# dmMaze/comic-text-detector

Measured on NVIDIA H100. Metric: pages/sec @1024x1024 synthetic, higher is better.
Workload: dtype fp16

## Files before the change

### comic-text-detector_b200/binding.py

```python
import collections
import ctypes as C
import os

import numpy as np

_HERE = os.path.dirname(os.path.abspath(__file__))
LIB_PATH = os.path.join(_HERE, "libctd_b200.so")
MAX_SRC = 3
ABI_VERSION = 3
PREC_FP16_TC, PREC_FP32_SIMT, PREC_FP16_SIMT, PREC_SPLIT_TC = 0, 1, 2, 3


class CtdOp(C.Structure):
    _fields_ = [("kind", C.c_int32), ("n_src", C.c_int32), ("src_buf", C.c_int32 * MAX_SRC),
                ("src_coff", C.c_int32 * MAX_SRC), ("src_c", C.c_int32 * MAX_SRC), ("dst_buf", C.c_int32),
                ("dst_coff", C.c_int32), ("cout", C.c_int32), ("cout_pad", C.c_int32), ("ksize", C.c_int32),
                ("stride", C.c_int32), ("act", C.c_int32), ("residual", C.c_int32), ("aux", C.c_int32),
                ("w16_off", C.c_int64), ("w32_off", C.c_int64), ("b_off", C.c_int64), ("p_off", C.c_int64)]


class CtdBufDesc(C.Structure):
    _fields_ = [("channels", C.c_int32), ("down", C.c_int32)]


class CtdConfig(C.Structure):
# ... 51 lines not shown
                ("event", C.c_void_p)]


class CtdNetOutput(C.Structure):
    _fields_ = [("blks", C.c_void_p), ("blks_stride_r", C.c_int64), ("blks_stride_c", C.c_int64),
                ("mask", C.c_void_p), ("mask_stride_h", C.c_int64), ("mask_stride_w", C.c_int64),
                ("lines", C.c_void_p), ("lines_stride_h", C.c_int64), ("lines_stride_w", C.c_int64),
                ("rows", C.c_int32), ("blks_on_device", C.c_int32), ("mask_on_device", C.c_int32),
                ("lines_on_device", C.c_int32), ("event", C.c_void_p)]


EXPORTS = ["ctd_create", "ctd_destroy", "ctd_last_error", "ctd_forward", "ctd_get_net_outputs", "ctd_get_mask_u8",
           "ctd_get_detections", "ctd_get_db_components", "ctd_last_forward_ms", "ctd_last_launch_count",
           "ctd_debug_read_buffer", "ctd_debug_write_buffer", "ctd_connected_components", "ctd_nms",
           "ctd_timer_start", "ctd_timer_stop", "ctd_profile_forward", "ctd_get_text_lines", "ctd_seg_represent",
           "ctd_refine_mask", "ctd_collect", "ctd_join", "ctd_resize_linear_u8", "ctd_debug_run_ops",
           "ctd_get_nms_status", "ctd_group_output", "ctd_detect_page", "ctd_results_layout", "ctd_submit_full",
           "ctd_device_arena", "ctd_region_plan", "ctd_transform_regions", "ctd_pages_plan", "ctd_submit_pages",
           "ctd_collect_regions", "ctd_collect_device", "ctd_forward_tensor", "ctd_jpeg_probe",
           "ctd_jpeg_decoder_create", "ctd_jpeg_decoder_destroy", "ctd_jpeg_decode", "ctd_debug_postprocess",
           "ctd_png_encoder_create", "ctd_png_encoder_destroy", "ctd_png_encode", "ctd_png_probe",
           "ctd_png_decoder_create", "ctd_png_decoder_destroy", "ctd_png_decode", "ctd_png_decoder_stats",
           "ctd_refine_plan", "ctd_submit_refine", "ctd_submit_regions", "ctd_debug_read_slot", "ctd_submit_outputs",
           "ctd_preprocess_pages", "ctd_submit_outputs_dtype", "ctd_forward_tensor_f16", "ctd_nms_dtype"]
PRE_F32_NCHW, PRE_F16_NCHW, PRE_U8_NHWC = 0, 1, 2
DTYPE_F32, DTYPE_F16 = 0, 1

_lib = None


class CtdError(RuntimeError):
# ... 39 lines not shown
    lib.ctd_debug_read_buffer.argtypes = [vp, i32, vp, C.c_size_t]
    lib.ctd_debug_write_buffer.argtypes = [vp, i32, vp, i32, i32, i32]
    lib.ctd_connected_components.argtypes = [vp, vp, i32, i32, vp, vp, i32, vp]
    lib.ctd_nms.argtypes = [vp, vp, i32, C.c_float, C.c_float, vp, vp]
    lib.ctd_nms_dtype.argtypes = [vp, vp, i32, i32, C.c_float, C.c_float, vp, vp]
    lib.ctd_get_text_lines.argtypes = [vp, vp, vp, vp]
    lib.ctd_seg_represent.argtypes = [vp, vp, i32, i32, C.c_float, vp, vp, vp]
    lib.ctd_refine_mask.argtypes = [vp, vp, vp, i32, i32, vp, i32, i32, vp]
    lib.ctd_timer_start.argtypes = [vp]
    lib.ctd_timer_stop.argtypes = [vp, C.POINTER(C.c_float)]
    lib.ctd_profile_forward.argtypes = [vp, vp, i32, i32, i32, i32, vp, i32]
    lib.ctd_collect.argtypes = [vp, i32]
    lib.ctd_join.argtypes = [vp, vp]
    lib.ctd_resize_linear_u8.argtypes = [vp, vp, i32, i32, i32, vp, i32, i32]
    lib.ctd_debug_run_ops.argtypes = [vp, vp, i32, i32, i32, i32, i32]
    lib.ctd_debug_postprocess.argtypes = [vp, vp, vp, i32, i32, i32]
    lib.ctd_get_nms_status.argtypes = [vp, vp, C.POINTER(i32)]
    lib.ctd_group_output.argtypes = [vp, vp, i32, vp, i32, i32, i32, vp, i32, vp, i32, vp, i32, vp, i32, C.POINTER(i32)]
    lib.ctd_detect_page.argtypes = [vp, vp, i32, i32, i32, i32, i32, i32, vp, vp, vp, i32, vp, i32, vp, i32, C.POINTER(i32)]
    lib.ctd_results_layout.argtypes = [vp, C.POINTER(CtdResultsLayout)]
    lib.ctd_submit_full.argtypes = [vp, i32, vp, i32, i32, i32, i32, i32, vp]
    lib.ctd_device_arena.argtypes = [vp, i32, C.POINTER(vp), C.POINTER(vp)]
    lib.ctd_region_plan.argtypes = [vp, i32, i32, i32, i32, vp, C.POINTER(C.c_size_t)]
    lib.ctd_transform_regions.argtypes = [vp, vp, i32, i32, i32, vp, i32, vp, C.c_size_t]
    lib.ctd_pages_plan.argtypes = [vp, i32, i32, i32, C.POINTER(C.c_size_t), C.POINTER(C.c_size_t)]
    lib.ctd_submit_pages.argtypes = [vp, i32, vp, i32, i32, i32, vp, vp, i32, i32, i32, i32, vp]
    lib.ctd_collect_regions.argtypes = [vp, i32, C.POINTER(vp), C.POINTER(i32), C.POINTER(vp), C.POINTER(vp),
                                        C.POINTER(C.c_size_t)]
    lib.ctd_collect_device.argtypes = [vp, i32, vp]
    lib.ctd_refine_plan.argtypes = [vp, i32, vp, vp, vp, vp, C.POINTER(C.c_size_t), C.POINTER(C.c_size_t)]
# ... 605 lines not shown
    def join(self, other):
        self._ck(self.lib.ctd_join(self.h, other.h))

    def debug_write(self, tensor, arr, n, h, w):
        arr = np.ascontiguousarray(arr, np.float32)
        ch = self.program.bufs[tensor["buf"]][0]
        assert arr.shape == (n, h // tensor["down"], w // tensor["down"], ch), arr.shape
        self._ck(self.lib.ctd_debug_write_buffer(self.h, tensor["buf"], _ptr(arr), n, h, w))

    def debug_run_ops(self, first, last, n, h, w, pages=None):
        if pages is not None:
            pages = np.ascontiguousarray(pages, dtype=np.uint8)
        self._ck(self.lib.ctd_debug_run_ops(self.h, _ptr(pages), n, h, w, first, last))
        self.shape = (n, h, w)

    def debug_read_slot(self, slot, plane, offset, nbytes):
        out = np.empty((nbytes,), np.uint8)
        self._ck(self.lib.ctd_debug_read_slot(self.h, slot, plane, offset, _ptr(out), nbytes))
        return out

    def debug_postprocess(self, blks, lines):
        blks = np.ascontiguousarray(blks, np.float32)
        lines = np.ascontiguousarray(lines, np.float32)
        n, c, h, w = lines.shape
        assert c == 2 and blks.shape == (n, 3 * ((h // 8) * (w // 8) + (h // 16) * (w // 16) + (h // 32) * (w // 32)),
                                         5 + self.nc), (blks.shape, lines.shape)
        self._ck(self.lib.ctd_debug_postprocess(self.h, _ptr(blks), _ptr(lines), n, h, w))
        self.shape = (n, h, w)

    def transform_regions(self, page, plan, out=None, page_shape=None):
# ... 34 lines not shown
```

### comic-text-detector_b200/csrc/conv_tc.cu

```cuda
#include <cstdlib>
#include <cstring>
#include <cuda.h>
#include <cuda_fp16.h>
#include <cuda_runtime.h>

#include "kernels.h"
#include "ptx.cuh"

namespace ctd {

constexpr int kTileW = 16;
constexpr int kThreads = 384;

template <int BN, int TH>
struct TcCfg {
  static constexpr int kABytes = TH * kTileW * 128;
  static constexpr int kBBytes = BN * 128;
  static constexpr int kStages = TH == 8 ? (BN >= 128 ? 5 : (BN >= 64 ? 8 : 10))
                                         : (BN >= 128 ? 3 : (BN >= 64 ? 4 : (BN >= 32 ? 5 : 6)));
  static constexpr int kBoxN = BN < 64 ? BN : 64;
  static constexpr int kBoxBytes = 8 * TH * kBoxN * 2;
  static constexpr int kStgBytes = (BN / kBoxN) * kBoxBytes;
  static constexpr int kBiasFloats = 512;
  static constexpr size_t kSmem = 1024 + size_t(kStages) * (kABytes + kBBytes) + 2 * kStgBytes + 256 + kBiasFloats * 4;
  static_assert(kSmem <= 227 * 1024, "conv_tc_kernel: shared memory");
  static_assert(kBoxBytes % 1024 == 0, "conv_tc_kernel: store boxes must keep the 1024-byte swizzle alignment");
};

template <int ACT>
__device__ __forceinline__ float apply_act(float v) {
  if constexpr (ACT == CTD_ACT_SILU) return __fdividef(v, 1.0f + exp_neg_fast(v));
  else if constexpr (ACT == CTD_ACT_LEAKY) return fmaxf(v, 0.1f * v);
  else if constexpr (ACT == CTD_ACT_RELU) return fmaxf(v, 0.f);
  else if constexpr (ACT == CTD_ACT_SIGMOID) return __fdividef(1.0f, 1.0f + exp_neg_fast(v));
  else return v;
}

template <int ACT>
__device__ __forceinline__ float apply_act_precise(float v) {
  if constexpr (ACT == CTD_ACT_SILU) return v / (1.0f + expf(-v));
  else if constexpr (ACT == CTD_ACT_LEAKY) return fmaxf(v, 0.1f * v);
  else if constexpr (ACT == CTD_ACT_RELU) return fmaxf(v, 0.f);
  else if constexpr (ACT == CTD_ACT_SIGMOID) return 1.0f / (1.0f + expf(-v));
  else return v;
}

template <int BN>
__device__ __forceinline__ void wgmma_bn(float (&d)[BN / 2], uint64_t ad, uint64_t bd, uint32_t acc) {
  if constexpr (BN == 128) wgmma_n128(d, ad, bd, acc);
  else if constexpr (BN == 64) wgmma_n64(d, ad, bd, acc);
  else if constexpr (BN == 32) wgmma_n32(d, ad, bd, acc);
  else wgmma_n16(d, ad, bd, acc);
}

template <int BN, int TH, int ACT, bool RES>
__device__ __forceinline__ void stage_f16(const float (&acc)[BN / 2], const float* __restrict__ bias_s, uint32_t stg,
                                          int m, int warp4, int lane) {
  using Cfg = TcCfg<BN, TH>;
  constexpr uint32_t kRowBytes = Cfg::kBoxN * 2;
  const int q = lane >> 3;
  const uint32_t pixrow = uint32_t(m * 64 + warp4 * 16 + (q & 1) * 8 + (lane & 7));
#pragma unroll
  for (int j = 0; j < BN / 8; j += 2) {
    const int col = (j + (q >> 1)) * 8;
    const uint32_t off = pixrow * kRowBytes + uint32_t(col % Cfg::kBoxN) * 2;
    const uint32_t addr = stg + uint32_t(col / Cfg::kBoxN) * Cfg::kBoxBytes +
                          (off ^ (((off >> 7) & (kRowBytes / 16 - 1)) << 4));
    uint32_t r[4];
    if constexpr (RES) ldmatrix_x4(addr, r);
#pragma unroll
    for (int i = 0; i < 4; ++i) {
      const int c = (j + (i >> 1)) * 8 + (lane & 3) * 2;
      float f0 = apply_act<ACT>(acc[j * 4 + 2 * i] + bias_s[c]);
      float f1 = apply_act<ACT>(acc[j * 4 + 2 * i + 1] + bias_s[c + 1]);
      if constexpr (RES) {
        __half2 h;
        memcpy(&h, &r[i], 4);
        const float2 rv = __half22float2(h);
        f0 = __fadd_rn(f0, rv.x);
        f1 = __fadd_rn(f1, rv.y);
      }
      const __half2 o = __floats2half2_rn(f0, f1);
      memcpy(&r[i], &o, 4);
    }
    stmatrix_x4(addr, r);
  }
}

template <int ACT>
__device__ __forceinline__ void epi_pair_f32(float v0, float v1, const float* __restrict__ bias_s, int col,
                                             float* __restrict__ out, int ncols, bool residual) {
  if (col >= ncols) return;
  float f0 = apply_act_precise<ACT>(v0 + bias_s[col]);
  float f1 = apply_act_precise<ACT>(v1 + bias_s[col + 1]);
  if (col + 1 < ncols) {
    if (residual) {
      const float2 r = *reinterpret_cast<const float2*>(out + col);
      f0 += r.x;
      f1 += r.y;
    }
    *reinterpret_cast<float2*>(out + col) = make_float2(f0, f1);
// ... 493 lines not shown
```

### comic-text-detector_b200/csrc/engine.cu

```cuda
#include <cuda.h>
#include <cuda_fp16.h>
#include <cuda_runtime.h>
#include <stdarg.h>
#include <stdio.h>
#include <string.h>

#include <algorithm>
#include <cstdlib>
#include <map>
#include <string>
#include <tuple>
#include <vector>

#include "engine.h"

using namespace ctd;

namespace {
thread_local std::string g_create_error;
}

int ctd_fail(ctd_handle* h, int code, const char* fmt, ...) {
  char buf[512];
  va_list ap;
// ... 131 lines not shown
  CKC(cudaEventCreate(&h->ev1));
  CKC(cudaEventCreate(&h->tev0));
  CKC(cudaEventCreate(&h->tev1));
  {
    void* fn = nullptr;
    cudaDriverEntryPointQueryResult qres;
    CKC(cudaGetDriverEntryPoint("cuTensorMapEncodeTiled", &fn, cudaEnableDefault, &qres));
    if (!fn || qres != cudaDriverEntryPointSuccess) {
      ctd_fail(h, CTD_E_CUDA, "cuTensorMapEncodeTiled not available from the driver");
      return bail(CTD_E_CUDA);
    }
    h->enc = reinterpret_cast<PFN_encodeTiled>(fn);
  }
  CKC(conv_tc_init());
  CKC(conv_ends_init());
  h->blob_bytes = blob_bytes;
  CKC(cudaMalloc(&h->d_blob, blob_bytes));
  CKC(cudaMemcpy(h->d_blob, blob, blob_bytes, cudaMemcpyHostToDevice));
  const size_t nb = size_t(cfg->max_batch), mh = cfg->max_h, mw = cfg->max_w;
  h->d_buf.assign(n_bufs, nullptr);
  for (int i = 0; i < n_bufs; ++i) {
    const size_t bytes = nb * (mh / bufs[i].down) * (mw / bufs[i].down + 4) * bufs[i].channels * h->elem;
    CKC(cudaMalloc(&h->d_buf[i], bytes));
    CKC(cudaMemset(h->d_buf[i], 0, bytes));
  }
  if (cfg->precision == CTD_PREC_SPLIT_TC) {
    h->d_buf16.assign(n_bufs, nullptr);
    for (int i = 0; i < n_bufs; ++i) {
      const size_t bytes = 2 * nb * (mh / bufs[i].down) * (mw / bufs[i].down + 4) * bufs[i].channels * 2;
      CKC(cudaMalloc(&h->d_buf16[i], bytes));
// ... 110 lines not shown
  p.det_stride = h->detect_prm[i][0];
  for (int k = 0; k < 6; ++k) p.anchor_wh[k] = h->detect_prm[i][1 + k];
}

static bool runs_on_tensor_cores(int precision, int kind) {
  switch (precision) {
    case CTD_PREC_SPLIT_TC: return is_gemm(kind);
    case CTD_PREC_FP16_TC: return is_gemm(kind) || kind == CTD_OP_STEM || kind == CTD_OP_SEG_TAIL;
    default: return false;
  }
}

static int build_plans(ctd_handle* h, int n, int ph, int pw, ShapePlan& sp) {
  sp.tc.resize(h->ops.size());
  sp.ends.resize(h->ops.size());
  const bool split = h->cfg.precision == CTD_PREC_SPLIT_TC;
  for (size_t i = 0; i < h->ops.size(); ++i) {
    const ctd_op& op = h->ops[i];
    if (!runs_on_tensor_cores(h->cfg.precision, op.kind)) continue;
    const float* bias = reinterpret_cast<const float*>(h->d_blob + op.b_off);
    const char* e = nullptr;
    if (op.kind == CTD_OP_STEM) {
      const bool f16 = sp.input == INPUT_F32;
      e = conv_ends_plan_stem(sp.ends[i], h->enc, f16 ? static_cast<const void*>(h->in_stage.p) : h->d_pages, f16, n,
                              ph, pw, h->d_blob + op.w16_off, bias, static_cast<__half*>(h->d_buf[op.dst_buf]),
                              h->bufs[op.dst_buf].channels, op.dst_coff, op.cout, op.act);
    } else if (op.kind == CTD_OP_SEG_TAIL) {
      if (op.cout_pad != 16) return ctd_fail(h, CTD_E_INVALID, "op %zu: seg tail needs cout_pad 16", i);
      const ctd_bufdesc& sb = h->bufs[op.src_buf[0]];
      e = conv_ends_plan_seg(sp.ends[i], h->enc, static_cast<const __half*>(h->d_buf[op.src_buf[0]]), sb.channels,
                             op.src_coff[0], op.src_c[0], n, ph / sb.down, pw / sb.down, h->d_blob + op.w16_off,
                             h->d_mask, h->d_mask_u8);
    } else {
      ConvGeom g;
      if (int rc = op_geom(h, op, n, ph, pw, g)) return rc;
      const void* src[CTD_MAX_SRC];
      int coff[CTD_MAX_SRC];
      for (int s = 0; s < op.n_src; ++s) {
        src[s] = (split ? h->d_buf16 : h->d_buf)[op.src_buf[s]];
        coff[s] = op.src_coff[s];
      }
      const void* w = split ? h->d_wsplit + h->wsplit_off[i] : h->d_blob + op.w16_off;
      __half* dst = op.kind == CTD_OP_DETECT ? nullptr : static_cast<__half*>(h->d_buf[op.dst_buf]);
      e = conv_tc_plan(sp.tc[i], h->enc, g, src, coff, w, bias, dst, split);
      if (op.kind == CTD_OP_DETECT) set_detect(h, i, ph, pw, sp.tc[i].p);
    }
    if (e) return ctd_fail(h, CTD_E_INVALID, "op %zu: %s", i, e);
  }
  return CTD_OK;
}

template <typename T>
static int run_op_simt(ctd_handle* h, size_t i, int n, int ph, int pw) {
  const ctd_op& op = h->ops[i];
  ConvSimtParams p;
  memset(&p, 0, sizeof(p));
  if (int rc = op_geom(h, op, n, ph, pw, p.g)) return rc;
  for (int k = 0; k < op.n_src; ++k)
    p.src[k] = static_cast<char*>(h->d_buf[op.src_buf[k]]) + size_t(op.src_coff[k]) * sizeof(T);
// ... 55 lines not shown
  else if (op.kind == CTD_OP_AVGPOOL2 || op.kind == CTD_OP_UPSAMPLE2) c = op.src_c[0];
  if (buf < 0 || c <= 0) return CTD_OK;
  const ctd_bufdesc& b = h->bufs[buf];
  const size_t npix = size_t(n) * (ph / b.down) * (pw / b.down);
  __half* hi = static_cast<__half*>(h->d_buf16[buf]) + coff;
  CK(split_planes_launch(static_cast<const float*>(h->d_buf[buf]) + coff, hi, hi + npix * b.channels, npix, c, b.channels,
                         h->stream));
  ++*cnt;
  return CTD_OK;
}

static int run_one_op(ctd_handle* h, size_t i, int n, int ph, int pw, const ShapePlan& sp, int* cnt) {
  const ctd_op& op = h->ops[i];
  const ConvTcPlan& tc = sp.tc[i];
  int rc = CTD_OK;
  if (tc.block_n || sp.ends[i].kind != ctd::CTD_END_NONE) {
    const cudaError_t e = tc.block_n ? conv_tc_launch(tc, h->stream) : conv_ends_launch(sp.ends[i], h->stream);
    if (e != cudaSuccess) rc = ctd_fail(h, CTD_E_CUDA, "tensor-core op %zu: %s", i, cudaGetErrorString(e));
  } else if (is_gemm(op.kind)) {
    rc = h->elem == 4 ? run_op_simt<float>(h, i, n, ph, pw) : run_op_simt<__half>(h, i, n, ph, pw);
  } else {
    rc = h->elem == 4 ? run_op_thin<float>(h, op, n, ph, pw, sp.input) : run_op_thin<__half>(h, op, n, ph, pw, sp.input);
  }
  ++*cnt;
  if (rc || h->d_buf16.empty()) return rc;
  return split_written_slice(h, op, n, ph, pw, cnt);
}

int launch_nms(ctd_handle* h, int n, int ph, int pw, cudaStream_t s, int* cnt, const int32_t* half) {
  CK(nms_launch(h->d_blks, n, rows_per_image(ph, pw), h->cfg.nc, h->cfg.conf_thresh, h->cfg.nms_thresh, h->nms, h->d_det,
                h->d_det_count, s, half));
  *cnt += kNmsLaunches;
// ... 432 lines not shown
  if (!h) return CTD_E_INVALID;
  if (first_op < 0 || last_op >= int(h->ops.size()) || first_op > last_op) return ctd_fail(h, CTD_E_INVALID, "bad op range");
  ShapePlan* sp = nullptr;
  if (int rc = find_plan(h, n, ph, pw, &sp)) return rc;
  if (pages) CK(cudaMemcpyAsync(h->d_pages, pages, size_t(n) * ph * pw * 3, cudaMemcpyHostToDevice, h->stream));
  int cnt = 0;
  for (int i = first_op; i <= last_op; ++i)
    if (int rc = run_one_op(h, size_t(i), n, ph, pw, *sp, &cnt)) return rc;
  CK(cudaStreamSynchronize(h->stream));
  h->n = n; h->ph = ph; h->pw = pw;
  h->have_forward = true;
  h->last_launches = cnt;
  return CTD_OK;
}

extern "C" int ctd_debug_postprocess(ctd_handle* h, const float* blks, const float* lines, int32_t n, int32_t ph,
                                     int32_t pw) {
  if (!h || !blks || !lines) return CTD_E_INVALID;
  if (h->cfg.debug_skip_postproc) return ctd_fail(h, CTD_E_INVALID, "ctd_debug_postprocess needs the full pipeline");
  ShapePlan* sp = nullptr;
  if (int rc = find_plan(h, n, ph, pw, &sp)) return rc;
  const size_t hw = size_t(ph) * pw;
  CK(cudaMemcpyAsync(h->d_blks, blks, size_t(n) * rows_per_image(ph, pw) * (5 + h->cfg.nc) * 4, cudaMemcpyHostToDevice,
                     h->stream));
  CK(cudaMemcpyAsync(h->d_lines, lines, size_t(n) * hw * 2 * 4, cudaMemcpyHostToDevice, h->stream));
  for (int i = 0; i < n; ++i)
    CK(binarize_launch(h->d_lines + size_t(i) * 2 * hw, hw, h->cfg.db_thresh, h->d_bitmap + size_t(i) * hw, h->stream));
  int cnt = 0;
  if (int rc = launch_nms(h, n, ph, pw, h->stream, &cnt)) return rc;
  if (int rc = launch_db_post(h, n, ph, pw, h->stream, &cnt)) return rc;
// ... 79 lines not shown
```

### comic-text-detector_b200/csrc/engine.h

```cpp
#pragma once
#include <cuda.h>
#include <cuda_runtime.h>
#include <stdint.h>

#include <math.h>

#include <algorithm>
#include <array>
#include <condition_variable>
#include <deque>
#include <map>
#include <mutex>
#include <optional>
#include <string>
#include <thread>
#include <tuple>
#include <vector>

#include "kernels.h"

using ctd::ConvTcPlan;
using ctd::ConvEndsPlan;
using ctd::NmsWorkspace;
using ctd::PFN_encodeTiled;

struct ArenaLayout {
  size_t det, cnt, nl, lb, ls, lc, a_bytes, refined, blocks, blocks_stride, rec_off, lines_off, dist_off, total;
};

struct BlockSection {
  size_t rec_off, lines_off, dist_off, stride;
};
inline BlockSection block_section_layout() {
  auto al = [](size_t v) { return (v + 255) / 256 * 256; };
  BlockSection b;
  b.rec_off = 64;
  b.lines_off = b.rec_off + al(size_t(CTD_MAX_BLOCKS) * sizeof(ctd_block));
// ... 113 lines not shown
struct RegionJob {
  std::vector<ctd::RegionDev> regs;
  std::vector<ctd::RegionTile> tiles;
  size_t out_bytes = 0;
  int add(const ctd_region* plan, int n, const ctd::RegionPage& pg, long long out_base);
  size_t table_bytes() const;
  void write_tables(char* dst) const;
};

enum { INPUT_U8 = 0, INPUT_F32 = 1 };

struct ShapePlan {
  int input = INPUT_U8;
  std::vector<ConvTcPlan> tc;
  std::vector<ConvEndsPlan> ends;
  cudaGraphExec_t graph = nullptr;
  int launches = 0;
};
struct ctd_handle {
  ctd_config cfg{};
  std::vector<ctd_op> ops;
  std::vector<ctd_bufdesc> bufs;
  std::vector<std::array<float, 7>> detect_prm;
  std::string err;
  cudaStream_t stream = nullptr;
  cudaEvent_t ev0 = nullptr, ev1 = nullptr, tev0 = nullptr, tev1 = nullptr;
  std::vector<cudaEvent_t> op_events;
  PFN_encodeTiled enc = nullptr;
  char* d_blob = nullptr;
  size_t blob_bytes = 0;
// ... 16 lines not shown
  void* d_segrep_scratch = nullptr;
  DevBuf refine_scratch;
  DevBuf cc_scratch;
  DevBuf io_scratch;
  int16_t* d_line_boxes = nullptr;
  float* d_line_scores = nullptr;
  int32_t* d_line_count = nullptr;
  void* d_nms_ws = nullptr;
  NmsWorkspace nms{};
  std::map<std::tuple<int, int, int, int>, ShapePlan> plans;
  DevBuf in_stage;
  cudaEvent_t ev_tin = nullptr, ev_tout = nullptr;
  cudaStream_t copy_in = nullptr, copy_out = nullptr;
  Slot slot[2];
  bool overlap = false;
  cudaStream_t side = nullptr, side2 = nullptr;
  cudaEvent_t ev_fork = nullptr, ev_join = nullptr, ev_fork2 = nullptr, ev_join2 = nullptr;
  cudaEvent_t ev_xjoin = nullptr;
  std::vector<char> db_ancestor;
  ArenaLayout layout{};
  cudaStream_t post = nullptr;
  size_t pipe_pinned_cap = 0;
  std::thread pipe_thread;
  std::mutex pipe_mu;
  std::condition_variable pipe_cv, pipe_done_cv;
  std::deque<PipeJob> pipe_queue;
  bool pipe_quit = false;
  int host_threads = 4;
  size_t pg_gather_off = 0;
  size_t pg_out_off = 0, pg_half_off = 0, pg_flag_off = 0;
// ... 24 lines not shown
```

### comic-text-detector_b200/csrc/kernels.h

```cpp
#pragma once
#include <cuda.h>
#include <cuda_fp16.h>
#include <cuda_runtime.h>
#include <stdint.h>

#include "../../include/ctd_b200.h"

namespace ctd {

constexpr int kMaxTaps = 9;

constexpr float kSplitLoScale = 2048.0f;
constexpr float kSplitLoUnscale = 1.0f / 2048.0f;
constexpr int kMaxPhases = 4;

struct ConvGeom {
  int n_img;
  int gh, gw;
  int dst_h, dst_w;
  int out_mul;
  int n_phase;
  int taps;
  int cin_total;
  int k_total;
// ... 40 lines not shown
  int block_n;
  int tile_h;
  dim3 grid;
  size_t smem_bytes;
};

typedef CUresult (*PFN_encodeTiled)(CUtensorMap*, CUtensorMapDataType, cuuint32_t, void*, const cuuint64_t*,
                                    const cuuint64_t*, const cuuint32_t*, const cuuint32_t*, CUtensorMapInterleave,
                                    CUtensorMapSwizzle, CUtensorMapL2promotion, CUtensorMapFloatOOBfill);

const char* conv_tc_plan(ConvTcPlan& plan, PFN_encodeTiled enc, const ConvGeom& g, const void* const src_ptr[],
                         const int src_coff[], const void* w16, const float* bias, __half* dst, int split = 0);
cudaError_t conv_tc_launch(const ConvTcPlan& plan, cudaStream_t s);
cudaError_t conv_tc_init();

enum { CTD_END_NONE = 0, CTD_END_STEM = 1, CTD_END_SEG = 2, CTD_END_STEM_F16 = 3 };
struct alignas(64) ConvEndsParams {
  CUtensorMap a_map;
  CUtensorMap b_map;
  CUtensorMap d_map;
  int n_img, gh, gw;
  int tiles_x, tiles_y;
  const float* bias;
  float* mask_f32;
  uint8_t* mask_u8;
};
struct ConvEndsPlan {
  ConvEndsParams p;
  int kind = CTD_END_NONE;
  dim3 grid;
// ... 148 lines not shown
```

### include/ctd_b200.h

```cpp
#ifndef CTD_B200_H_
#define CTD_B200_H_

#include <stddef.h>
#include <stdint.h>

#ifdef __cplusplus
extern "C" {
#endif

#define CTD_ABI_VERSION 3
#if defined(__GNUC__)
#define CTD_API __attribute__((visibility("default")))
#else
#define CTD_API
#endif

#define CTD_OK 0
#define CTD_E_INVALID (-1)
#define CTD_E_CUDA (-2)
#define CTD_E_NO_DEVICE (-3)
#define CTD_E_SHAPE (-4)
#define CTD_E_CAPACITY (-5)


// ... 86 lines not shown

CTD_API int ctd_get_text_lines(ctd_handle* h, int16_t* boxes, float* scores, int32_t* counts);

CTD_API int ctd_resize_linear_u8(ctd_handle* h, const uint8_t* src, int32_t sh, int32_t sw, int32_t channels, uint8_t* dst,
                                 int32_t dh, int32_t dw);

CTD_API int ctd_join(ctd_handle* h, ctd_handle* other);

CTD_API int ctd_last_forward_ms(ctd_handle* h, float* ms);
CTD_API int ctd_last_launch_count(ctd_handle* h, int32_t* launches);
CTD_API int ctd_debug_read_buffer(ctd_handle* h, int32_t buf, float* out, size_t out_elems);
CTD_API int ctd_debug_write_buffer(ctd_handle* h, int32_t buf, const float* in, int32_t n, int32_t ph, int32_t pw);

CTD_API int ctd_debug_run_ops(ctd_handle* h, const uint8_t* pages, int32_t n, int32_t ph, int32_t pw, int32_t first_op,
                              int32_t last_op);

CTD_API int ctd_debug_postprocess(ctd_handle* h, const float* blks, const float* lines, int32_t n, int32_t ph, int32_t pw);

CTD_API int ctd_debug_read_slot(ctd_handle* h, int32_t slot, int32_t plane, size_t offset, uint8_t* out, size_t bytes);

CTD_API int ctd_timer_start(ctd_handle* h);
CTD_API int ctd_timer_stop(ctd_handle* h, float* ms);
CTD_API int ctd_profile_forward(ctd_handle* h, const uint8_t* pages, int32_t n, int32_t ph, int32_t pw,
                                int32_t pages_on_device, float* op_ms, int32_t cap);

CTD_API int ctd_connected_components(ctd_handle* h, const uint8_t* img, int32_t ih, int32_t iw, int32_t* labels,
                             int32_t* stats, int32_t stats_cap, int32_t* n_labels);

CTD_API int ctd_seg_represent(ctd_handle* h, const float* pred, int32_t ih, int32_t iw, float thresh, int16_t* boxes,
                              float* scores, int32_t* count);
// ... 220 lines not shown
```

Baseline: 1149.

## Add persistent warp-specialized pointwise conv kernel with weights resident in shared memory

Adds a dedicated 1x1 convolution kernel that loads the full weight slice for its output-channel block into shared memory once, then runs persistent CTAs. Two producer warps stream activation tiles through TMA rings feeding two consumer warpgroups that use wgmma, with a TMA-store epilogue. Eligible 1x1 convs go to it by default (can be disabled with an env var) and the shared epilogue helpers move into a common header. The goal is to avoid reloading weights per tile and to overlap loads with MMA. The cost is a larger shared-memory footprint and one CTA per SM, and layers that don't meet the size or alignment checks fall back to the old kernel.

Result: no change. 1158 (median of 6 runs) (+0.8%).

```diff
diff --git a/comic-text-detector_b200/binding.py b/comic-text-detector_b200/binding.py
--- a/comic-text-detector_b200/binding.py
+++ b/comic-text-detector_b200/binding.py
@@ -9,6 +9,7 @@
 MAX_SRC = 3
 ABI_VERSION = 3
 PREC_FP16_TC, PREC_FP32_SIMT, PREC_FP16_SIMT, PREC_SPLIT_TC = 0, 1, 2, 3
+KERNEL_CUDA_CORES, KERNEL_CONV_TC, KERNEL_ENDS, KERNEL_CONV_PW = 0, 1, 2, 3
 
 
 class CtdOp(C.Structure):
@@ -90,7 +91,7 @@
            "ctd_get_detections", "ctd_get_db_components", "ctd_last_forward_ms", "ctd_last_launch_count",
            "ctd_debug_read_buffer", "ctd_debug_write_buffer", "ctd_connected_components", "ctd_nms",
            "ctd_timer_start", "ctd_timer_stop", "ctd_profile_forward", "ctd_get_text_lines", "ctd_seg_represent",
-           "ctd_refine_mask", "ctd_collect", "ctd_join", "ctd_resize_linear_u8", "ctd_debug_run_ops",
+           "ctd_refine_mask", "ctd_collect", "ctd_join", "ctd_resize_linear_u8", "ctd_debug_run_ops", "ctd_debug_op_kernel",
            "ctd_get_nms_status", "ctd_group_output", "ctd_detect_page", "ctd_results_layout", "ctd_submit_full",
            "ctd_device_arena", "ctd_region_plan", "ctd_transform_regions", "ctd_pages_plan", "ctd_submit_pages",
            "ctd_collect_regions", "ctd_collect_device", "ctd_forward_tensor", "ctd_jpeg_probe",
@@ -160,6 +161,7 @@
     lib.ctd_join.argtypes = [vp, vp]
     lib.ctd_resize_linear_u8.argtypes = [vp, vp, i32, i32, i32, vp, i32, i32]
     lib.ctd_debug_run_ops.argtypes = [vp, vp, i32, i32, i32, i32, i32]
+    lib.ctd_debug_op_kernel.argtypes = [vp, i32, i32, i32, i32, C.POINTER(i32), C.POINTER(i32)]
     lib.ctd_debug_postprocess.argtypes = [vp, vp, vp, i32, i32, i32]
     lib.ctd_get_nms_status.argtypes = [vp, vp, C.POINTER(i32)]
     lib.ctd_group_output.argtypes = [vp, vp, i32, vp, i32, i32, i32, vp, i32, vp, i32, vp, i32, vp, i32, C.POINTER(i32)]
@@ -795,6 +797,11 @@
         self._ck(self.lib.ctd_debug_run_ops(self.h, _ptr(pages), n, h, w, first, last))
         self.shape = (n, h, w)
 
+    def debug_op_kernel(self, op, n, h, w):
+        kernel, bn = C.c_int32(), C.c_int32()
+        self._ck(self.lib.ctd_debug_op_kernel(self.h, n, h, w, op, C.byref(kernel), C.byref(bn)))
+        return kernel.value, bn.value
+
     def debug_read_slot(self, slot, plane, offset, nbytes):
         out = np.empty((nbytes,), np.uint8)
         self._ck(self.lib.ctd_debug_read_slot(self.h, slot, plane, offset, _ptr(out), nbytes))
diff --git a/comic-text-detector_b200/csrc/conv_epi.cuh b/comic-text-detector_b200/csrc/conv_epi.cuh
--- /dev/null
+++ b/comic-text-detector_b200/csrc/conv_epi.cuh
@@ -0,0 +1,68 @@
+#pragma once
+#include <cstring>
+#include <cuda_fp16.h>
+
+#include "kernels.h"
+#include "ptx.cuh"
+
+namespace ctd {
+
+template <int ACT>
+__device__ __forceinline__ float apply_act(float v) {
+  if constexpr (ACT == CTD_ACT_SILU) return __fdividef(v, 1.0f + exp_neg_fast(v));
+  else if constexpr (ACT == CTD_ACT_LEAKY) return fmaxf(v, 0.1f * v);
+  else if constexpr (ACT == CTD_ACT_RELU) return fmaxf(v, 0.f);
+  else if constexpr (ACT == CTD_ACT_SIGMOID) return __fdividef(1.0f, 1.0f + exp_neg_fast(v));
+  else return v;
+}
+
+template <int BN>
+__device__ __forceinline__ void wgmma_bn(float (&d)[BN / 2], uint64_t ad, uint64_t bd, uint32_t acc) {
+  if constexpr (BN == 128) wgmma_n128(d, ad, bd, acc);
+  else if constexpr (BN == 64) wgmma_n64(d, ad, bd, acc);
+  else if constexpr (BN == 32) wgmma_n32(d, ad, bd, acc);
+  else wgmma_n16(d, ad, bd, acc);
+}
+
+template <int BN, int TH>
+struct StgCfg {
+  static constexpr int kBoxN = BN < 64 ? BN : 64;
+  static constexpr int kBoxBytes = 8 * TH * kBoxN * 2;
+  static constexpr int kBytes = (BN / kBoxN) * kBoxBytes;
+};
+
+template <int BN, int TH, int ACT, bool RES>
+__device__ __forceinline__ void stage_f16(const float (&acc)[BN / 2], const float* __restrict__ bias_s, uint32_t stg,
+                                          int m, int warp4, int lane) {
+  using Cfg = StgCfg<BN, TH>;
+  constexpr uint32_t kRowBytes = Cfg::kBoxN * 2;
+  const int q = lane >> 3;
+  const uint32_t pixrow = uint32_t(m * 64 + warp4 * 16 + (q & 1) * 8 + (lane & 7));
+#pragma unroll
+  for (int j = 0; j < BN / 8; j += 2) {
+    const int col = (j + (q >> 1)) * 8;
+    const uint32_t off = pixrow * kRowBytes + uint32_t(col % Cfg::kBoxN) * 2;
+    const uint32_t addr = stg + uint32_t(col / Cfg::kBoxN) * Cfg::kBoxBytes +
+                          (off ^ (((off >> 7) & (kRowBytes / 16 - 1)) << 4));
+    uint32_t r[4];
+    if constexpr (RES) ldmatrix_x4(addr, r);
+#pragma unroll
+    for (int i = 0; i < 4; ++i) {
+      const int c = (j + (i >> 1)) * 8 + (lane & 3) * 2;
+      float f0 = apply_act<ACT>(acc[j * 4 + 2 * i] + bias_s[c]);
+      float f1 = apply_act<ACT>(acc[j * 4 + 2 * i + 1] + bias_s[c + 1]);
+      if constexpr (RES) {
+        __half2 h;
+        memcpy(&h, &r[i], 4);
+        const float2 rv = __half22float2(h);
+        f0 = __fadd_rn(f0, rv.x);
+        f1 = __fadd_rn(f1, rv.y);
+      }
+      const __half2 o = __floats2half2_rn(f0, f1);
+      memcpy(&r[i], &o, 4);
+    }
+    stmatrix_x4(addr, r);
+  }
+}
+
+}
diff --git a/comic-text-detector_b200/csrc/conv_pw.cu b/comic-text-detector_b200/csrc/conv_pw.cu
--- /dev/null
+++ b/comic-text-detector_b200/csrc/conv_pw.cu
@@ -0,0 +1,273 @@
+#include <cstring>
+#include <cuda.h>
+#include <cuda_fp16.h>
+#include <cuda_runtime.h>
+
+#include "conv_epi.cuh"
+#include "kernels.h"
+#include "ptx.cuh"
+
+namespace ctd {
+
+namespace {
+
+constexpr int kThreads = 384;
+constexpr int kTileW = 16, kTileH = 8;
+constexpr int kRows = kTileW * kTileH;
+constexpr int kMinStages = 3, kMaxStages = 4;
+constexpr size_t kSmemMax = 227 * 1024;
+constexpr uint32_t kBarBytes = 256;
+
+size_t smem_bytes(int bn, int kb, int k_total, int stages) {
+  return 1024 + size_t(bn) * k_total * 2 + size_t(2 * stages) * kRows * kb * 2 + 2 * size_t(kRows) * bn * 2 + kBarBytes +
+         size_t(bn) * 4;
+}
+
+int g_sms = 132;
+
+}
+
+template <int BN, int ACT>
+__global__ void __launch_bounds__(kThreads, 1) conv_pw_kernel(const __grid_constant__ ConvPwParams p) {
+  using Stg = StgCfg<BN, 2 * kTileH>;
+  static_assert(Stg::kBoxN == 64 && Stg::kBytes == kRows * BN * 2, "conv_pw_kernel: staging boxes");
+  extern __shared__ __align__(1024) uint8_t smem_pw[];
+  const uint32_t raw = smem_u32(smem_pw);
+  const uint32_t base = (raw + 1023u) & ~1023u;
+  uint8_t* const gen = smem_pw + (base - raw);
+  const int kb = p.kb, nkb = p.n_kblocks, S = p.stages;
+  const uint32_t row_bytes = uint32_t(kb) * 2;
+  const uint32_t w_box = BN * row_bytes, a_stage = kRows * row_bytes;
+  const uint32_t w_base = base;
+  const uint32_t a_base = w_base + uint32_t(nkb) * w_box;
+  const uint32_t stg_base = a_base + uint32_t(2 * S) * a_stage;
+  const uint32_t bar = stg_base + 2 * Stg::kBytes;
+  const uint32_t full_bar = bar, empty_bar = bar + 16 * S, w_bar = bar + 32 * S;
+  float* const bias_s = reinterpret_cast<float*>(gen + (bar - base) + kBarBytes);
+
+  const int warp = threadIdx.x >> 5, lane = threadIdx.x & 31;
+  const int nblk = blockIdx.x % p.n_nblk, member = blockIdx.x / p.n_nblk;
+
+  if (threadIdx.x == 0) {
+    for (int s = 0; s < p.n_src; ++s) prefetch_tensormap(&p.a_map[s]);
+    prefetch_tensormap(&p.b_map);
+    prefetch_tensormap(&p.d_map);
+    for (int s = 0; s < 2 * S; ++s) {
+      mbar_init(full_bar + 8 * s, 1);
+      mbar_init(empty_bar + 8 * s, 1);
+    }
+    mbar_init(w_bar, 1);
+    fence_barrier_init();
+  }
+  for (int i = threadIdx.x; i < BN; i += kThreads) bias_s[i] = p.bias ? p.bias[nblk * BN + i] : 0.f;
+  __syncthreads();
+
+  auto decode = [&](int t, int& img, int& y0, int& x0) {
+    const int tiles_per_img = p.tiles_x * p.tiles_y;
+    img = t / tiles_per_img;
+    const int r = t - img * tiles_per_img;
+    const int ty = r / p.tiles_x;
+    y0 = ty * kTileH;
+    x0 = (r - ty * p.tiles_x) * kTileW;
+  };
+
+  if (warp < 4) {
+    setmaxnreg_dec<40>();
+    if (warp < 2 && elect_one()) {
+      if (warp == 0) {
+        mbar_arrive_expect_tx(w_bar, uint32_t(nkb) * w_box);
+        for (int k = 0; k < nkb; ++k) tma_load_2d(w_base + k * w_box, &p.b_map, w_bar, k * kb, nblk * BN);
+      }
+      const uint32_t ring = a_base + uint32_t(warp * S) * a_stage;
+      const uint32_t full = full_bar + 8 * warp * S, empty = empty_bar + 8 * warp * S;
+      int it = 0;
+      for (int t = member + warp * p.members; t < p.spatial; t += 2 * p.members) {
+        int img, y0, x0;
+        decode(t, img, y0, x0);
+        for (int s = 0; s < p.n_src; ++s)
+          for (int cb = 0; cb < p.src_kblocks[s]; ++cb, ++it) {
+            const int stage = it % S;
+            mbar_wait_relaxed(empty + 8 * stage, ((it / S) & 1) ^ 1);
+            mbar_arrive_expect_tx(full + 8 * stage, a_stage);
+            tma_load_4d(ring + stage * a_stage, &p.a_map[s], full + 8 * stage, cb * kb, x0, y0, img);
+          }
+      }
+    }
+    return;
+  }
+
+  setmaxnreg_inc<232>();
+  const int wg = (warp >> 2) - 1;
+  const bool leader = (threadIdx.x & 127) == 0;
+  const uint32_t ring = a_base + uint32_t(wg * S) * a_stage;
+  const uint32_t full = full_bar + 8 * wg * S, empty = empty_bar + 8 * wg * S;
+  const uint64_t a_desc0 = make_kmajor_desc(ring, row_bytes);
+  const uint64_t b_desc0 = make_kmajor_desc(w_base, row_bytes);
+  const uint64_t a_mstep = (64u * row_bytes) >> 4;
+  const int ksteps = kb / 16;
+  const uint32_t stg = stg_base + uint32_t(wg) * Stg::kBytes;
+  const uint32_t epi_bar = 1 + wg;
+  constexpr int R = BN / 2;
+  int stage = 0;
+  uint32_t full_par = 0;
+  mbar_wait(w_bar, 0);
+
+  for (int t = member + wg * p.members; t < p.spatial; t += 2 * p.members) {
+    float acc[2][R];
+#pragma unroll
+    for (int m = 0; m < 2; ++m)
+#pragma unroll
+      for (int i = 0; i < R; ++i) acc[m][i] = 0.f;
+    int prev = -1;
+    for (int k = 0; k < nkb; ++k) {
+      mbar_wait(full + 8 * stage, full_par);
+      const uint64_t ad = a_desc0 + uint64_t(stage) * (a_stage >> 4);
+      const uint64_t bd = b_desc0 + uint64_t(k) * (w_box >> 4);
+      wgmma_fence();
+      for (int ks = 0; ks < ksteps; ++ks)
+#pragma unroll
+        for (int m = 0; m < 2; ++m)
+          wgmma_bn<BN>(acc[m], ad + m * a_mstep + 2 * ks, bd + 2 * ks, (k > 0 || ks > 0) ? 1u : 0u);
+      wgmma_commit();
+      wgmma_wait<1>();
+      if (prev >= 0 && leader) mbar_arrive(empty + 8 * prev);
+      prev = stage;
+      if (++stage == S) { stage = 0; full_par ^= 1u; }
+    }
+    wgmma_wait<0>();
+#pragma unroll
+    for (int m = 0; m < 2; ++m) wgmma_fence_regs(acc[m]);
+    if (prev >= 0 && leader) mbar_arrive(empty + 8 * prev);
+
+    if (leader) tma_store_wait_read();
+    named_barrier_sync(epi_bar, 128);
+#pragma unroll
+    for (int m = 0; m < 2; ++m) stage_f16<BN, 2 * kTileH, ACT, false>(acc[m], bias_s, stg, m, warp & 3, lane);
+    fence_proxy_async();
+    named_barrier_sync(epi_bar, 128);
+    if (leader) {
+      int img, y0, x0;
+      decode(t, img, y0, x0);
+#pragma unroll
+      for (int b = 0; b < BN / 64; ++b) tma_store_4d(&p.d_map, stg + b * Stg::kBoxBytes, nblk * BN + b * 64, x0, y0, img);
+      tma_store_commit();
+    }
+  }
+  if (leader) tma_store_wait_all();
+}
+
+
+namespace {
+
+const char* encode(PFN_encodeTiled enc, CUtensorMap* m, const void* base, int rank, const cuuint64_t* dims,
+                   const cuuint64_t* strides_bytes, const cuuint32_t* box, int kb_elems) {
+  const cuuint32_t estr[4] = {1, 1, 1, 1};
+  const CUtensorMapSwizzle sw = kb_elems == 64 ? CU_TENSOR_MAP_SWIZZLE_128B
+                                               : (kb_elems == 32 ? CU_TENSOR_MAP_SWIZZLE_64B : CU_TENSOR_MAP_SWIZZLE_32B);
+  const CUresult r = enc(m, CU_TENSOR_MAP_DATA_TYPE_FLOAT16, rank, const_cast<void*>(base), dims, strides_bytes, box,
+                         estr, CU_TENSOR_MAP_INTERLEAVE_NONE, sw, CU_TENSOR_MAP_L2_PROMOTION_L2_256B,
+                         CU_TENSOR_MAP_FLOAT_OOB_FILL_NONE);
+  return r == CUDA_SUCCESS ? nullptr : "cuTensorMapEncodeTiled failed";
+}
+
+int conv_pw_stages(int bn, int kb, int k_total) {
+  int s = kMaxStages;
+  while (s >= kMinStages && smem_bytes(bn, kb, k_total, s) > kSmemMax) --s;
+  return s >= kMinStages ? s : 0;
+}
+
+constexpr int kMinTilesPerCta = 3;
+
+}
+
+const char* conv_pw_plan(ConvPwPlan& plan, PFN_encodeTiled enc, const ConvGeom& g, const void* const src_ptr[],
+                         const int src_coff[], const void* w16, const float* bias, __half* dst) {
+  ConvPwParams& p = plan.p;
+  memset(&p, 0, sizeof(p));
+  plan.block_n = 0;
+  if (g.taps != 1 || g.in_stride != 1 || g.n_phase != 1 || dst == nullptr || g.residual != 0) return nullptr;
+  if (g.cout_pad % 64 != 0 || g.cout % 8 != 0 || g.dst_coff % 8 != 0 || g.dst_cstride % 8 != 0) return nullptr;
+  if (g.act < CTD_ACT_NONE || g.act > CTD_ACT_SIGMOID) return nullptr;
+  int kb = 64;
+  for (int s = 0; s < g.n_src; ++s) {
+    if (g.src_c[s] % 64 != 0 && kb > 32) kb = 32;
+    if (g.src_c[s] % 32 != 0) kb = 16;
+    if (g.src_c[s] % 16 != 0 || src_coff[s] % 8 != 0) return nullptr;
+  }
+  const int bn = g.cout_pad % 128 == 0 ? 128 : 64;
+  const int stages = conv_pw_stages(bn, kb, g.k_total);
+  if (stages == 0) return nullptr;
+  p.n_img = g.n_img;
+  p.tiles_x = (g.gw + kTileW - 1) / kTileW;
+  p.tiles_y = (g.gh + kTileH - 1) / kTileH;
+  p.n_nblk = g.cout_pad / bn;
+  p.spatial = g.n_img * p.tiles_x * p.tiles_y;
+  p.members = g_sms / p.n_nblk > 0 ? g_sms / p.n_nblk : 1;
+  if (p.spatial < kMinTilesPerCta * p.members) return nullptr;
+  p.n_src = g.n_src;
+  p.kb = kb;
+  p.n_kblocks = g.k_total / kb;
+  for (int s = 0; s < g.n_src; ++s) p.src_kblocks[s] = g.src_c[s] / kb;
+  p.stages = stages;
+  p.act = g.act;
+  p.bias = bias;
+  for (int s = 0; s < g.n_src; ++s) {
+    const cuuint64_t cs = cuuint64_t(g.src_cstride[s]) * 2;
+    const char* b = static_cast<const char*>(src_ptr[s]) + size_t(src_coff[s]) * 2;
+    const cuuint64_t dims[4] = {cuuint64_t(g.src_c[s]), cuuint64_t(g.src_w), cuuint64_t(g.src_h), cuuint64_t(g.n_img)};
+    const cuuint64_t str[3] = {cs, cs * g.src_w, cs * g.src_w * g.src_h};
+    const cuuint32_t box[4] = {cuuint32_t(kb), kTileW, kTileH, 1};
+    if (const char* e = encode(enc, &p.a_map[s], b, 4, dims, str, box, kb)) return e;
+  }
+  {
+    const cuuint64_t dims[2] = {cuuint64_t(g.k_total), cuuint64_t(g.cout_pad)};
+    const cuuint64_t str[1] = {cuuint64_t(g.k_total) * 2};
+    const cuuint32_t box[2] = {cuuint32_t(kb), cuuint32_t(bn)};
+    if (const char* e = encode(enc, &p.b_map, w16, 2, dims, str, box, kb)) return e;
+  }
+  {
+    const cuuint64_t px = cuuint64_t(g.dst_cstride) * 2;
+    const cuuint64_t dims[4] = {cuuint64_t(g.cout), cuuint64_t(g.gw), cuuint64_t(g.gh), cuuint64_t(g.n_img)};
+    const cuuint64_t str[3] = {px, px * g.dst_w, px * g.dst_w * g.dst_h};
+    const cuuint32_t box[4] = {64, kTileW, kTileH, 1};
+    if (const char* e = encode(enc, &p.d_map, reinterpret_cast<const char*>(dst) + size_t(g.dst_coff) * 2, 4, dims,
+                               str, box, 64))
+      return e;
+  }
+  plan.block_n = bn;
+  plan.grid = dim3(unsigned(p.members * p.n_nblk), 1, 1);
+  plan.smem_bytes = smem_bytes(bn, kb, g.k_total, stages);
+  return nullptr;
+}
+
+#define CTD_PW_INSTANCES(X)                                                                                     \
+  X(128, CTD_ACT_NONE) X(128, CTD_ACT_SILU) X(128, CTD_ACT_LEAKY) X(128, CTD_ACT_RELU) X(128, CTD_ACT_SIGMOID) \
+  X(64, CTD_ACT_NONE) X(64, CTD_ACT_SILU) X(64, CTD_ACT_LEAKY) X(64, CTD_ACT_RELU) X(64, CTD_ACT_SIGMOID)
+
+cudaError_t conv_pw_init() {
+  int dev = 0;
+  if (cudaGetDevice(&dev) == cudaSuccess) {
+    int n = 0;
+    if (cudaDeviceGetAttribute(&n, cudaDevAttrMultiProcessorCount, dev) == cudaSuccess && n > 0) g_sms = n;
+  }
+  cudaError_t e;
+#define CTD_SET(BN, ACT)                                                                                          \
+  e = cudaFuncSetAttribute(conv_pw_kernel<BN, ACT>, cudaFuncAttributeMaxDynamicSharedMemorySize, int(kSmemMax)); \
+  if (e != cudaSuccess) return e;
+  CTD_PW_INSTANCES(CTD_SET)
+#undef CTD_SET
+  return cudaSuccess;
+}
+
+cudaError_t conv_pw_launch(const ConvPwPlan& plan, cudaStream_t s) {
+#define CTD_LAUNCH(BN, ACT)                                                               \
+  if (plan.block_n == BN && plan.p.act == ACT) {                                          \
+    conv_pw_kernel<BN, ACT><<<plan.grid, kThreads, plan.smem_bytes, s>>>(plan.p);         \
+    return cudaGetLastError();                                                            \
+  }
+  CTD_PW_INSTANCES(CTD_LAUNCH)
+#undef CTD_LAUNCH
+  return cudaErrorInvalidValue;
+}
+
+}
diff --git a/comic-text-detector_b200/csrc/conv_tc.cu b/comic-text-detector_b200/csrc/conv_tc.cu
--- a/comic-text-detector_b200/csrc/conv_tc.cu
+++ b/comic-text-detector_b200/csrc/conv_tc.cu
@@ -4,6 +4,7 @@
 #include <cuda_fp16.h>
 #include <cuda_runtime.h>
 
+#include "conv_epi.cuh"
 #include "kernels.h"
 #include "ptx.cuh"
 
@@ -18,23 +19,14 @@
   static constexpr int kBBytes = BN * 128;
   static constexpr int kStages = TH == 8 ? (BN >= 128 ? 5 : (BN >= 64 ? 8 : 10))
                                          : (BN >= 128 ? 3 : (BN >= 64 ? 4 : (BN >= 32 ? 5 : 6)));
-  static constexpr int kBoxN = BN < 64 ? BN : 64;
-  static constexpr int kBoxBytes = 8 * TH * kBoxN * 2;
-  static constexpr int kStgBytes = (BN / kBoxN) * kBoxBytes;
+  static constexpr int kBoxN = StgCfg<BN, TH>::kBoxN;
+  static constexpr int kBoxBytes = StgCfg<BN, TH>::kBoxBytes;
+  static constexpr int kStgBytes = StgCfg<BN, TH>::kBytes;
   static constexpr int kBiasFloats = 512;
   static constexpr size_t kSmem = 1024 + size_t(kStages) * (kABytes + kBBytes) + 2 * kStgBytes + 256 + kBiasFloats * 4;
   static_assert(kSmem <= 227 * 1024, "conv_tc_kernel: shared memory");
   static_assert(kBoxBytes % 1024 == 0, "conv_tc_kernel: store boxes must keep the 1024-byte swizzle alignment");
 };
-
-template <int ACT>
-__device__ __forceinline__ float apply_act(float v) {
-  if constexpr (ACT == CTD_ACT_SILU) return __fdividef(v, 1.0f + exp_neg_fast(v));
-  else if constexpr (ACT == CTD_ACT_LEAKY) return fmaxf(v, 0.1f * v);
-  else if constexpr (ACT == CTD_ACT_RELU) return fmaxf(v, 0.f);
-  else if constexpr (ACT == CTD_ACT_SIGMOID) return __fdividef(1.0f, 1.0f + exp_neg_fast(v));
-  else return v;
-}
 
 template <int ACT>
 __device__ __forceinline__ float apply_act_precise(float v) {
@@ -43,48 +35,6 @@
   else if constexpr (ACT == CTD_ACT_RELU) return fmaxf(v, 0.f);
   else if constexpr (ACT == CTD_ACT_SIGMOID) return 1.0f / (1.0f + expf(-v));
   else return v;
-}
-
-template <int BN>
-__device__ __forceinline__ void wgmma_bn(float (&d)[BN / 2], uint64_t ad, uint64_t bd, uint32_t acc) {
-  if constexpr (BN == 128) wgmma_n128(d, ad, bd, acc);
-  else if constexpr (BN == 64) wgmma_n64(d, ad, bd, acc);
-  else if constexpr (BN == 32) wgmma_n32(d, ad, bd, acc);
-  else wgmma_n16(d, ad, bd, acc);
-}
-
-template <int BN, int TH, int ACT, bool RES>
-__device__ __forceinline__ void stage_f16(const float (&acc)[BN / 2], const float* __restrict__ bias_s, uint32_t stg,
-                                          int m, int warp4, int lane) {
-  using Cfg = TcCfg<BN, TH>;
-  constexpr uint32_t kRowBytes = Cfg::kBoxN * 2;
-  const int q = lane >> 3;
-  const uint32_t pixrow = uint32_t(m * 64 + warp4 * 16 + (q & 1) * 8 + (lane & 7));
-#pragma unroll
-  for (int j = 0; j < BN / 8; j += 2) {
-    const int col = (j + (q >> 1)) * 8;
-    const uint32_t off = pixrow * kRowBytes + uint32_t(col % Cfg::kBoxN) * 2;
-    const uint32_t addr = stg + uint32_t(col / Cfg::kBoxN) * Cfg::kBoxBytes +
-                          (off ^ (((off >> 7) & (kRowBytes / 16 - 1)) << 4));
-    uint32_t r[4];
-    if constexpr (RES) ldmatrix_x4(addr, r);
-#pragma unroll
-    for (int i = 0; i < 4; ++i) {
-      const int c = (j + (i >> 1)) * 8 + (lane & 3) * 2;
-      float f0 = apply_act<ACT>(acc[j * 4 + 2 * i] + bias_s[c]);
-      float f1 = apply_act<ACT>(acc[j * 4 + 2 * i + 1] + bias_s[c + 1]);
-      if constexpr (RES) {
-        __half2 h;
-        memcpy(&h, &r[i], 4);
-        const float2 rv = __half22float2(h);
-        f0 = __fadd_rn(f0, rv.x);
-        f1 = __fadd_rn(f1, rv.y);
-      }
-      const __half2 o = __floats2half2_rn(f0, f1);
-      memcpy(&r[i], &o, 4);
-    }
-    stmatrix_x4(addr, r);
-  }
 }
 
 template <int ACT>
diff --git a/comic-text-detector_b200/csrc/engine.cu b/comic-text-detector_b200/csrc/engine.cu
--- a/comic-text-detector_b200/csrc/engine.cu
+++ b/comic-text-detector_b200/csrc/engine.cu
@@ -169,6 +169,11 @@
   }
   CKC(conv_tc_init());
   CKC(conv_ends_init());
+  CKC(conv_pw_init());
+  {
+    const char* pw = getenv("CTD_CONV_PW");
+    h->conv_pw = !(pw && strcmp(pw, "0") == 0);
+  }
   h->blob_bytes = blob_bytes;
   CKC(cudaMalloc(&h->d_blob, blob_bytes));
   CKC(cudaMemcpy(h->d_blob, blob, blob_bytes, cudaMemcpyHostToDevice));
@@ -309,6 +314,7 @@
 static int build_plans(ctd_handle* h, int n, int ph, int pw, ShapePlan& sp) {
   sp.tc.resize(h->ops.size());
   sp.ends.resize(h->ops.size());
+  sp.pw.resize(h->ops.size());
   const bool split = h->cfg.precision == CTD_PREC_SPLIT_TC;
   for (size_t i = 0; i < h->ops.size(); ++i) {
     const ctd_op& op = h->ops[i];
@@ -337,7 +343,9 @@
       }
       const void* w = split ? h->d_wsplit + h->wsplit_off[i] : h->d_blob + op.w16_off;
       __half* dst = op.kind == CTD_OP_DETECT ? nullptr : static_cast<__half*>(h->d_buf[op.dst_buf]);
-      e = conv_tc_plan(sp.tc[i], h->enc, g, src, coff, w, bias, dst, split);
+      if (!split && h->conv_pw && op.kind == CTD_OP_CONV && op.ksize == 1)
+        e = conv_pw_plan(sp.pw[i], h->enc, g, src, coff, w, bias, dst);
+      if (!e && !sp.pw[i].block_n) e = conv_tc_plan(sp.tc[i], h->enc, g, src, coff, w, bias, dst, split);
       if (op.kind == CTD_OP_DETECT) set_detect(h, i, ph, pw, sp.tc[i].p);
     }
     if (e) return ctd_fail(h, CTD_E_INVALID, "op %zu: %s", i, e);
@@ -423,8 +431,10 @@
   const ctd_op& op = h->ops[i];
   const ConvTcPlan& tc = sp.tc[i];
   int rc = CTD_OK;
-  if (tc.block_n || sp.ends[i].kind != ctd::CTD_END_NONE) {
-    const cudaError_t e = tc.block_n ? conv_tc_launch(tc, h->stream) : conv_ends_launch(sp.ends[i], h->stream);
+  if (tc.block_n || sp.pw[i].block_n || sp.ends[i].kind != ctd::CTD_END_NONE) {
+    const cudaError_t e = tc.block_n         ? conv_tc_launch(tc, h->stream)
+                          : sp.pw[i].block_n ? conv_pw_launch(sp.pw[i], h->stream)
+                                             : conv_ends_launch(sp.ends[i], h->stream);
     if (e != cudaSuccess) rc = ctd_fail(h, CTD_E_CUDA, "tensor-core op %zu: %s", i, cudaGetErrorString(e));
   } else if (is_gemm(op.kind)) {
     rc = h->elem == 4 ? run_op_simt<float>(h, i, n, ph, pw) : run_op_simt<__half>(h, i, n, ph, pw);
@@ -887,6 +897,20 @@
   return CTD_OK;
 }
 
+extern "C" int ctd_debug_op_kernel(ctd_handle* h, int32_t n, int32_t ph, int32_t pw, int32_t op, int32_t* kernel,
+                                   int32_t* block_n) {
+  if (!h || !kernel || !block_n) return CTD_E_INVALID;
+  if (op < 0 || op >= int(h->ops.size())) return ctd_fail(h, CTD_E_INVALID, "bad op index");
+  ShapePlan* sp = nullptr;
+  if (int rc = find_plan(h, n, ph, pw, &sp)) return rc;
+  const size_t i = size_t(op);
+  if (sp->pw[i].block_n) { *kernel = CTD_KERNEL_CONV_PW; *block_n = sp->pw[i].block_n; }
+  else if (sp->tc[i].block_n) { *kernel = CTD_KERNEL_CONV_TC; *block_n = sp->tc[i].block_n; }
+  else if (sp->ends[i].kind != ctd::CTD_END_NONE) { *kernel = CTD_KERNEL_ENDS; *block_n = 0; }
+  else { *kernel = CTD_KERNEL_CUDA_CORES; *block_n = 0; }
+  return CTD_OK;
+}
+
 extern "C" int ctd_debug_postprocess(ctd_handle* h, const float* blks, const float* lines, int32_t n, int32_t ph,
                                      int32_t pw) {
   if (!h || !blks || !lines) return CTD_E_INVALID;
diff --git a/comic-text-detector_b200/csrc/engine.h b/comic-text-detector_b200/csrc/engine.h
--- a/comic-text-detector_b200/csrc/engine.h
+++ b/comic-text-detector_b200/csrc/engine.h
@@ -21,6 +21,7 @@
 
 using ctd::ConvTcPlan;
 using ctd::ConvEndsPlan;
+using ctd::ConvPwPlan;
 using ctd::NmsWorkspace;
 using ctd::PFN_encodeTiled;
 
@@ -164,6 +165,7 @@
   int input = INPUT_U8;
   std::vector<ConvTcPlan> tc;
   std::vector<ConvEndsPlan> ends;
+  std::vector<ConvPwPlan> pw;
   cudaGraphExec_t graph = nullptr;
   int launches = 0;
 };
@@ -210,6 +212,7 @@
   cudaStream_t copy_in = nullptr, copy_out = nullptr;
   Slot slot[2];
   bool overlap = false;
+  bool conv_pw = true;
   cudaStream_t side = nullptr, side2 = nullptr;
   cudaEvent_t ev_fork = nullptr, ev_join = nullptr, ev_fork2 = nullptr, ev_join2 = nullptr;
   cudaEvent_t ev_xjoin = nullptr;
diff --git a/comic-text-detector_b200/csrc/kernels.h b/comic-text-detector_b200/csrc/kernels.h
--- a/comic-text-detector_b200/csrc/kernels.h
+++ b/comic-text-detector_b200/csrc/kernels.h
@@ -78,6 +78,34 @@
 cudaError_t conv_tc_launch(const ConvTcPlan& plan, cudaStream_t s);
 cudaError_t conv_tc_init();
 
+struct alignas(64) ConvPwParams {
+  CUtensorMap a_map[CTD_MAX_SRC];
+  CUtensorMap b_map;
+  CUtensorMap d_map;
+  int n_img, tiles_x, tiles_y;
+  int n_src;
+  int src_kblocks[CTD_MAX_SRC];
+  int kb;
+  int n_kblocks;
+  int stages;
+  int n_nblk;
+  int members;
+  int spatial;
+  int act;
+  const float* bias;
+};
+static_assert(sizeof(ConvPwParams) <= 4096, "ConvPwParams: kernel parameters are limited to 4 KB");
+struct ConvPwPlan {
+  ConvPwParams p;
+  int block_n = 0;
+  dim3 grid;
+  size_t smem_bytes;
+};
+const char* conv_pw_plan(ConvPwPlan& plan, PFN_encodeTiled enc, const ConvGeom& g, const void* const src_ptr[],
+                         const int src_coff[], const void* w16, const float* bias, __half* dst);
+cudaError_t conv_pw_launch(const ConvPwPlan& plan, cudaStream_t s);
+cudaError_t conv_pw_init();
+
 enum { CTD_END_NONE = 0, CTD_END_STEM = 1, CTD_END_SEG = 2, CTD_END_STEM_F16 = 3 };
 struct alignas(64) ConvEndsParams {
   CUtensorMap a_map;
diff --git a/include/ctd_b200.h b/include/ctd_b200.h
--- a/include/ctd_b200.h
+++ b/include/ctd_b200.h
@@ -124,6 +124,10 @@
 
 CTD_API int ctd_debug_run_ops(ctd_handle* h, const uint8_t* pages, int32_t n, int32_t ph, int32_t pw, int32_t first_op,
                               int32_t last_op);
+
+enum ctd_kernel { CTD_KERNEL_CUDA_CORES = 0, CTD_KERNEL_CONV_TC = 1, CTD_KERNEL_ENDS = 2, CTD_KERNEL_CONV_PW = 3 };
+CTD_API int ctd_debug_op_kernel(ctd_handle* h, int32_t n, int32_t ph, int32_t pw, int32_t op, int32_t* kernel,
+                                int32_t* block_n);
 
 CTD_API int ctd_debug_postprocess(ctd_handle* h, const float* blks, const float* lines, int32_t n, int32_t ph, int32_t pw);
 
```
